# circletile/smvp-toolkit

Measured on AMD Instinct MI355X. Metric: fp64 CSR SpMV GFLOP/s (2*nnz flop per product; achieved HBM GB/s in roofline), higher is better.
Workload: dtype f64; 1 GPU; memplus.mtx x944 block-diagonal (substitute for the SURVEY 8(d) random model; that model: roofline.frac_sur...; format=csr, kernel=csr_stream_owner<8, 5, false>, nnz=119085600, rows=16763552, exchange=none

## Files before the change

### smvp-toolkit_amd/csrc/smvp_kernels.hip

```cpp
#include "smvp_kernels.h"

#include <algorithm>
#include <cstdio>
#include <cstdlib>

namespace smvp {

template <int WIDTH>
__device__ __forceinline__ double shfl_down_sum(double v)
{
#pragma unroll
    for (int off = WIDTH / 2; off > 0; off >>= 1)
        v += __shfl_down(v, off, WIDTH);
    return v;
}


#ifndef SMVP_TU_ILP
template <int T>
__global__ __launch_bounds__(kVectorBlock) void csr_vector_rows(
    const int *__restrict__ row_ptr, const int *__restrict__ col_ind, const double *__restrict__ val,
    const double *__restrict__ x, double *__restrict__ y, int rows, int row0)
{
    const long long gid = (long long)blockIdx.x * kVectorBlock + threadIdx.x;
    const long long row = row0 + gid / T;
    const int lane = threadIdx.x & (T - 1);
    int a = 0, z = 0;
    if (row < rows) {
        a = row_ptr[row];
        z = row_ptr[row + 1];
    }
    double acc = 0.0;
    for (int j = a + lane; j < z; j += T)
        acc += val[j] * x[col_ind[j]];
    acc = shfl_down_sum<T>(acc);
    if (lane == 0 && row < rows)
        y[row] = acc;
}

template <int VPT>
__global__ __launch_bounds__(kStreamBlock) void csr_stream_tiles(
    const int *__restrict__ row_ptr, const int *__restrict__ col_ind, const double *__restrict__ val,
    const double *__restrict__ x, double *__restrict__ y, const int *__restrict__ tile_row,
    double *__restrict__ carry, int rows, int nnz, int ntiles, int tile_group)
{
    constexpr int TILE = kStreamBlock * VPT;
    constexpr int QCAP = TILE / kLongRow + 1;
    __shared__ double prod[TILE];
    __shared__ int long_rows[QCAP];
    __shared__ int long_count;

    const int b = tile_of_block(blockIdx.x, tile_group);
    if (b >= ntiles)
        return;
    const int t = threadIdx.x;
    const long long s = (long long)b * TILE;
    const int e = (int)(s + TILE < (long long)nnz ? s + TILE : (long long)nnz);
    if (t == 0)
        long_count = 0;
    const int rlo = tile_row[b];
    const int rhi = tile_row[b + 1];

    const long long j0 = s + (long long)t * VPT;
    double p[VPT];
    if (j0 + VPT <= (long long)nnz) {
        int c[VPT];
        double v[VPT];
#pragma unroll
        for (int k = 0; k < VPT; k += 4)
            *reinterpret_cast<int4 *>(&c[k]) = *reinterpret_cast<const int4 *>(col_ind + j0 + k);
#pragma unroll
        for (int k = 0; k < VPT; k += 2)
            *reinterpret_cast<double2 *>(&v[k]) = *reinterpret_cast<const double2 *>(val + j0 + k);
#pragma unroll
        for (int k = 0; k < VPT; ++k)
            p[k] = v[k] * x[c[k]];
    } else {
#pragma unroll
        for (int k = 0; k < VPT; ++k)
            p[k] = (j0 + k < (long long)nnz) ? val[j0 + k] * x[col_ind[j0 + k]] : 0.0;
    }
#pragma unroll
    for (int k = 0; k < VPT; k += 2)
        *reinterpret_cast<double2 *>(&prod[t * VPT + k]) = make_double2(p[k], p[k + 1]);
    __syncthreads();

    const int lo = (int)s;
    if (t < 64) {
        const int first = rlo < rows ? row_ptr[rlo] : nnz;
        const int head = (first < e ? first : e) - lo;
        double acc = 0.0;
        for (int i = t; i < head; i += 64)
            acc += prod[i];
        acc = shfl_down_sum<64>(acc);
        if (t == 0)
            carry[b] = acc;
    }

    for (int r = rlo + t; r < rhi; r += kStreamBlock) {
        const int a = row_ptr[r];
        const int nxt = row_ptr[r + 1];
        const int z = nxt < e ? nxt : e;
        if (z - a <= kLongRow) {
            double acc = 0.0;
            for (int i = a - lo; i < z - lo; ++i)
                acc += prod[i];
            y[r] = acc;
        } else {
            long_rows[atomicAdd(&long_count, 1)] = r;
        }
    }
    __syncthreads();

    const int nlong = long_count;
    const int lane = t & 63;
    for (int q = t >> 6; q < nlong; q += kStreamBlock / 64) {
        const int r = long_rows[q];
        const int a = row_ptr[r];
        const int nxt = row_ptr[r + 1];
        const int z = nxt < e ? nxt : e;
        double acc = 0.0;
        for (int i = a - lo + lane; i < z - lo; i += 64)
            acc += prod[i];
        acc = shfl_down_sum<64>(acc);
        if (lane == 0)
            y[r] = acc;
    }
}

#endif
typedef int int4v __attribute__((ext_vector_type(4)));

struct OwnerExtra {
    const int *pos = nullptr;
    const int *start_pos = nullptr;
    const int *ovf_ptr = nullptr;
    const double *ovf_val = nullptr;
    const int *ovf_k = nullptr;
    const int *cache_ptr = nullptr;
    const double *val_cache = nullptr;
    const unsigned short *col16 = nullptr;
    const int *col_base = nullptr;
    const unsigned *word32 = nullptr;
    const unsigned short *group_run = nullptr;
    const int *run_ptr = nullptr;
    const int *run_tab = nullptr;
    int unit_x = 0;
    const unsigned short *row_rel = nullptr;
    unsigned long long *stamps = nullptr;
    int back_grid = 0;
};

[[maybe_unused]] static inline OwnerExtra owner_extra_of(const OwnerLaunch &l, unsigned long long *stamps)
{
    OwnerExtra ex{};
    ex.pos = l.pos, ex.start_pos = l.start_pos, ex.ovf_ptr = l.ovf_ptr, ex.ovf_val = l.ovf_val, ex.ovf_k = l.ovf_k;
    ex.cache_ptr = l.cache_ptr, ex.val_cache = l.val_cache;
    ex.col16 = l.col16, ex.col_base = l.col_base;
    ex.unit_x = l.unit_x, ex.word32 = l.word32, ex.group_run = l.group_run, ex.run_ptr = l.run_ptr, ex.run_tab = l.run_tab;
    ex.row_rel = l.row_rel;
    ex.stamps = stamps;
    return ex;
}

struct OwnerArgs {
    const int *__restrict__ col_ind;
    const double *__restrict__ val;
    const double *__restrict__ x;
    const int *__restrict__ pos;
    const int *__restrict__ start_pos;
    const double *__restrict__ ovf_val;
    const int *__restrict__ ovf_k;
    int unit_x;
};

template <int FLAVOR>
__device__ __forceinline__ double owner_product_slow(const OwnerArgs &a, long long j)
{
    if constexpr (FLAVOR == kFlavorCsr || FLAVOR == kFlavorCsr16)
        return a.val[j] * a.x[a.col_ind[j]];
    else if constexpr (FLAVOR == kFlavorTjdsK)
        return a.val[a.pos[j]] * a.x[a.col_ind[j]];
    else {
        const int p = a.pos[j];
        return a.val[p] * a.x[p - a.start_pos[(unsigned)a.col_ind[j] >> kSlotBits]];
    }
}

template <int FLAVOR>
__device__ __forceinline__ double owner_overflow_product(const OwnerArgs &a, int ovf_base, int e, int i)
{
    if constexpr (FLAVOR == kFlavorTjdsS || FLAVOR == kFlavorTjdsH)
        return a.unit_x ? a.val[a.ovf_k[ovf_base + i]] : a.ovf_val[ovf_base + i] * a.x[a.ovf_k[ovf_base + i]];
    else
        return owner_product_slow<FLAVOR>(a, (long long)e + i);
}

#if defined(SMVP_PHASE_STAMPS) && defined(SMVP_TU_ILP)
#undef SMVP_PHASE_STAMPS
#define SMVP_ILP_UNIT_UNUSED
#endif
#ifdef SMVP_PHASE_STAMPS
__device__ unsigned long long g_owner_phase[8];
#define SMVP_PHASE(n)                                                                        \
    do {                                                                                     \
        if (threadIdx.x == 0 && (blockIdx.x & 127) == 5) {                                   \
            const unsigned long long now_ = wall_clock64();                                  \
            if ((n) > 0)                                                                     \
                atomicAdd(&g_owner_phase[(n)-1], now_ - phase_prev_);                        \
            else                                                                             \
                atomicAdd(&g_owner_phase[7], 1ull);                                          \
            phase_prev_ = now_;                                                              \
        }                                                                                    \
    } while (0)
#else
#define SMVP_PHASE(n) do { } while (0)
#endif

#ifndef SMVP_TJDS_NEUTRALISE
#define SMVP_TJDS_NEUTRALISE 0
#endif

template <int VPT, int FLAVOR, bool STAMPED>
__device__ __forceinline__ void owner_body(
    const int *__restrict__ row_ptr, const int *__restrict__ col_ind, const double *__restrict__ val,
    const double *__restrict__ x, double *__restrict__ y, const int *__restrict__ tile_row,
    const int *__restrict__ tile_next, int rows, int nnz_arg, int ntiles, int tile_group_arg, const OwnerExtra &ex, const int block)
{
    const OwnerArgs a = {col_ind, val, x, ex.pos, ex.start_pos, ex.ovf_val, ex.ovf_k, FLAVOR == kFlavorTjdsH ? ex.unit_x : 0};
    constexpr int TILE = kStreamBlock * VPT;
    constexpr int QCAP = (TILE + kStreamOver) / kLongRow + 1;
    constexpr bool CSR = FLAVOR == kFlavorCsr || FLAVOR == kFlavorCsr16;
    constexpr bool COL16 = FLAVOR == kFlavorCsr16;
    constexpr bool HALF = FLAVOR == kFlavorTjdsH;
    constexpr bool TJDS = FLAVOR == kFlavorTjdsK || FLAVOR == kFlavorTjdsS || HALF;
    constexpr bool SORTED = FLAVOR == kFlavorTjdsS || HALF;
    static_assert(TILE <= (1 << kSlotBits), "slot bits");
    __shared__ double prod[TILE + kStreamOver];
    __shared__ int long_rows[QCAP];
    __shared__ int long_a[QCAP];
    __shared__ int long_z[QCAP];
    __shared__ int long_count;
    __shared__ double wave_sum[kStreamBlock / 64];

    const int t = threadIdx.x;
#ifdef SMVP_PHASE_STAMPS
    unsigned long long phase_prev_ = 0;
#endif
    unsigned long long *stamp = nullptr;
    if constexpr (STAMPED) {
        stamp = ex.stamps + 2 * ((size_t)block * (kStreamBlock / 64) + (t >> 6));
        if ((t & 63) == 0)
            stamp[0] = wall_clock64();
    }
#define SMVP_OWNER_EXIT()                                         \
    do {                                                          \
        if constexpr (STAMPED) {                                  \
            asm volatile("s_waitcnt vmcnt(0)" ::: "memory");      \
            if ((t & 63) == 0)                                    \
                stamp[1] = wall_clock64();                        \
        }                                                         \
        return;                                                   \
    } while (0)

    const int b = tile_of_block_swept(block, tile_group_arg, ex.back_grid);
    if (b >= ntiles)
        SMVP_OWNER_EXIT();
    const int nnz = nnz_arg;
    const long long s = (long long)b * TILE;
    const long long j0 = s + (long long)t * VPT;

    const bool whole = j0 + VPT <= (long long)nnz;
    int c[VPT];
    int pj[VPT];
    double v[VPT];
    const bool full_tile = s + TILE <= (long long)nnz;
    int grp[HALF ? VPT : 1];
    int run0 = 0;
    int2 run_tbl = make_int2(0, 0);
    if constexpr (HALF) {
        if (full_tile) {
            run0 = ex.run_ptr[b];
            const int nruns = ex.run_ptr[b + 1] - run0;
            const int ln = t & 63;
            if (ln < nruns)
                run_tbl = reinterpret_cast<const int2 *>(ex.run_tab)[run0 + ln];
        }
    }
    if constexpr (HALF) {
        if (full_tile) {
#pragma unroll
            for (int k = 0; k < VPT; ++k) {
                if constexpr (VPT == 1) {
                    pj[k] = (int)ex.word32[s + k * kStreamBlock + t];
                } else {
                    pj[k] = (int)__builtin_nontemporal_load(ex.word32 + s + k * kStreamBlock + t);
                }
                const unsigned gw = reinterpret_cast<const unsigned *>(ex.group_run)[((size_t)b * (TILE / 32) + k * (kStreamBlock / 32) +
                                                                                     2 * __builtin_amdgcn_readfirstlane(t >> 6)) >> 1];
                grp[k] = (t & 32) ? (int)(gw >> 16) : (int)(gw & 0xffffu);
            }
        }
    } else if constexpr (SORTED) {
        if (full_tile) {
#pragma unroll
            for (int k = 0; k < VPT; ++k) {
                if constexpr (VPT > 1) {
                    pj[k] = __builtin_nontemporal_load(a.pos + s + k * kStreamBlock + t);
                    c[k] = __builtin_nontemporal_load(a.col_ind + s + k * kStreamBlock + t);
                } else {
                    pj[k] = a.pos[s + k * kStreamBlock + t];
                    c[k] = a.col_ind[s + k * kStreamBlock + t];
                }
            }
        }
    } else if (whole) {
        if constexpr (VPT >= 4) {
            if constexpr (COL16) {
                const int base = ex.col_base[b];
                if (base >= 0) {
#pragma unroll
                    for (int k = 0; k < VPT; k += 4) {
                        const uint2 w = *reinterpret_cast<const uint2 *>(ex.col16 + j0 + k);
                        c[k] = base + (int)(w.x & 0xffffu), c[k + 1] = base + (int)(w.x >> 16);
                        c[k + 2] = base + (int)(w.y & 0xffffu), c[k + 3] = base + (int)(w.y >> 16);
                    }
                } else {
#pragma unroll
                    for (int k = 0; k < VPT; k += 4)
                        *reinterpret_cast<int4 *>(&c[k]) = *reinterpret_cast<const int4 *>(a.col_ind + j0 + k);
                }
            } else {
#pragma unroll
                for (int k = 0; k < VPT; k += 4)
                    *reinterpret_cast<int4 *>(&c[k]) = *reinterpret_cast<const int4 *>(a.col_ind + j0 + k);
            }
            if constexpr (TJDS) {
#pragma unroll
                for (int k = 0; k < VPT; k += 4)
                    *reinterpret_cast<int4v *>(&pj[k]) = __builtin_nontemporal_load(reinterpret_cast<const int4v *>(a.pos + j0 + k));
            }
            if constexpr (CSR) {
#pragma unroll
                for (int k = 0; k < VPT; k += 2)
                    *reinterpret_cast<double2 *>(&v[k]) = *reinterpret_cast<const double2 *>(a.val + j0 + k);
            }
        } else {
            c[0] = a.col_ind[j0];
            if constexpr (TJDS)
                pj[0] = a.pos[j0];
            if constexpr (CSR)
                v[0] = a.val[j0];
        }
    }
    const int rlo = tile_row[b];
    const int rhi = tile_row[b + 1];
    if (rlo == rhi)
        SMVP_OWNER_EXIT();
    SMVP_PHASE(0);
    const int lo = (int)s;
    const int e = (int)(s + TILE < (long long)nnz ? s + TILE : (long long)nnz);
    const int zend = tile_next[b];
    const int ext = zend - e;
    const unsigned short *__restrict__ row_rel = ex.row_rel;
    auto row_bounds = [&](int r, int &ra, int &rz) {
        if (row_rel) {
            ra = row_rel[r];
            rz = r + 1 < rhi ? (int)row_rel[r + 1] : zend - lo;
        } else {
            ra = row_ptr[r] - lo;
            rz = row_ptr[r + 1] - lo;
        }
    };
    const bool giant = ext > kStreamOver;
    if (t == 0)
        long_count = 0;
    const bool over0 = !giant && t < ext;
    double p[VPT];
    double po = 0.0;
    int rp_a = 0, rp_b = 0, rp_a2 = 0, rp_b2 = 0;
    int ovf_base = 0, cache0 = 0, in_place = 0;
    if constexpr (SORTED) {
        ovf_base = ex.ovf_ptr[b];
        cache0 = ex.cache_ptr[b];
        in_place = (e - lo) - (ex.cache_ptr[b + 1] - cache0);
    }
    if constexpr (SORTED) {
        if (full_tile && rlo + t < rhi)
            row_bounds(rlo + t, rp_a, rp_b);
        if (full_tile && rlo + t + kStreamBlock < rhi)
            row_bounds(rlo + t + kStreamBlock, rp_a2, rp_b2);
        int co = 0;
        double vo = 0.0;
        const bool unit_x = HALF && ex.unit_x;
        if (over0 && !(SMVP_TJDS_NEUTRALISE & 8)) {
            co = a.ovf_k[ovf_base + t];
            if (!unit_x)
                vo = a.ovf_val[ovf_base + t];
        }
        if (full_tile) {
            int slot[VPT];
#pragma unroll
            for (int k = 0; k < VPT; ++k) {
                if constexpr (HALF)
                    c[k] = (int)((unsigned)pj[k] >> 16), pj[k] &= 0xffff;
                slot[k] = c[k] & ((1 << kSlotBits) - 1);
                if constexpr (HALF) {
                    const int r = grp[k] + (((c[k] >> kSlotBits) - grp[k]) & 31);
                    int base = __shfl(run_tbl.x, r & 63), sub = __shfl(run_tbl.y, r & 63);
                    if (r >= 64) {
                        const int2 w = reinterpret_cast<const int2 *>(ex.run_tab)[run0 + r];
                        base = w.x, sub = w.y;
                    }
                    pj[k] += base;
                    c[k] = pj[k] - sub;
                } else {
                    c[k] = pj[k] - a.start_pos[(unsigned)c[k] >> kSlotBits];
                }
            }
            double xk[VPT];
#pragma unroll
            for (int k = 0; k < VPT; ++k) {
                const int idx = k * kStreamBlock + t;
                const double *src = idx < in_place ? a.val + pj[k] : ex.val_cache + (cache0 + (idx - in_place));
                if ((SMVP_TJDS_NEUTRALISE & 2) && idx < in_place)
                    v[k] = 1.0;
                else if ((SMVP_TJDS_NEUTRALISE & 4) && idx >= in_place)
                    v[k] = 1.0;
                else
                    v[k] = *src;
            }
            double xo = 0.0;
            if (unit_x) {
#pragma unroll
                for (int k = 0; k < VPT; ++k)
                    xk[k] = 1.0;
                if (over0)
                    vo = a.val[co], xo = 1.0;
            } else {
#pragma unroll
                for (int k = 0; k < VPT; ++k)
                    xk[k] = (SMVP_TJDS_NEUTRALISE & 1) ? 1.0 : a.x[c[k]];
                xo = over0 && !(SMVP_TJDS_NEUTRALISE & 8) ? a.x[co] : 0.0;
            }
#pragma unroll
            for (int k = 0; k < VPT; ++k)
                prod[slot[k]] = v[k] * xk[k];
            po = vo * xo;
        } else {
            for (int k = 0; k < VPT; ++k) {
                const int idx = k * kStreamBlock + t;
                if (s + idx < (long long)nnz) {
                    if constexpr (HALF) {
                        const unsigned w32 = ex.word32[s + idx];
                        const int m = (int)(w32 >> 16), g = ex.group_run[(size_t)b * (TILE / 32) + (idx >> 5)];
                        const int r = g + (((m >> kSlotBits) - g) & 31);
                        const int2 w = reinterpret_cast<const int2 *>(ex.run_tab)[ex.run_ptr[b] + r];
                        const int pw = w.x + (int)(w32 & 0xffffu);
                        const double vv = idx < in_place ? a.val[pw] : ex.val_cache[cache0 + (idx - in_place)];
                        prod[m & ((1 << kSlotBits) - 1)] = unit_x ? vv : vv * a.x[pw - w.y];
                    } else {
                        const int pw = a.pos[s + idx];
                        const double vv = idx < in_place ? a.val[pw] : ex.val_cache[cache0 + (idx - in_place)];
                        const int m = a.col_ind[s + idx];
                        prod[m & ((1 << kSlotBits) - 1)] = vv * a.x[pw - a.start_pos[(unsigned)m >> kSlotBits]];
                    }
                }
            }
            if (over0)
                po = unit_x ? a.val[co] : vo * a.x[co];
        }
    } else if (whole) {
        if (rlo + t < rhi)
            row_bounds(rlo + t, rp_a, rp_b);
        if (rlo + t + kStreamBlock < rhi)
            row_bounds(rlo + t + kStreamBlock, rp_a2, rp_b2);
        int co = 0, pjo = 0;
        double vo = 0.0;
        if (over0) {
            co = a.col_ind[e + t];
            if constexpr (TJDS)
                pjo = a.pos[e + t];
            if constexpr (CSR)
                vo = a.val[e + t];
        }
        double xk[VPT];
        if constexpr (TJDS) {
#pragma unroll
            for (int k = 0; k < VPT; ++k)
                v[k] = a.val[pj[k]];
            if (over0)
                vo = a.val[pjo];
        }
#pragma unroll
        for (int k = 0; k < VPT; ++k)
            xk[k] = a.x[c[k]];
        const double xo = over0 ? a.x[co] : 0.0;
#pragma unroll
        for (int k = 0; k < VPT; ++k)
            p[k] = v[k] * xk[k];
        po = vo * xo;
    } else {
#pragma unroll
        for (int k = 0; k < VPT; ++k)
            p[k] = (j0 + k < (long long)nnz) ? owner_product_slow<FLAVOR>(a, j0 + k) : 0.0;
        if (over0)
            po = owner_product_slow<FLAVOR>(a, e + t);
    }
    if constexpr (!SORTED) {
        if constexpr (VPT >= 2) {
#pragma unroll
            for (int k = 0; k < VPT; k += 2)
                *reinterpret_cast<double2 *>(&prod[t * VPT + k]) = make_double2(p[k], p[k + 1]);
        } else {
            prod[t] = p[0];
        }
    }
    if (over0)
        prod[e - lo + t] = po;
    if (!giant)
        for (int i = t + kStreamBlock; i < ext; i += kStreamBlock)
            prod[e - lo + i] = owner_overflow_product<FLAVOR>(a, ovf_base, e, i);
    SMVP_PHASE(1);
    __syncthreads();
    SMVP_PHASE(2);

    const int last = rhi - 1;
    auto finish_row = [&](int r, int ra, int rz) {
        if (rz - ra <= kLongRow) {
            double acc = 0.0;
            for (int i = ra; i < rz; i += 4) {
                const double v0 = prod[i], v1 = prod[i + 1 < rz ? i + 1 : i], v2 = prod[i + 2 < rz ? i + 2 : i],
                             v3 = prod[i + 3 < rz ? i + 3 : i];
                acc += v0;
                if (i + 1 < rz)
                    acc += v1;
                if (i + 2 < rz)
                    acc += v2;
                if (i + 3 < rz)
                    acc += v3;
            }
            if constexpr (VPT == 1)
                y[r] = acc;
            else
                __builtin_nontemporal_store(acc, &y[r]);
        } else {
            const int q = atomicAdd(&long_count, 1);
            long_rows[q] = r;
            long_a[q] = ra;
            long_z[q] = rz;
        }
    };
    int r_next = rlo + t;
    if (full_tile) {
        if (r_next < rhi && !(giant && r_next == last))
            finish_row(r_next, rp_a, rp_b);
        r_next += kStreamBlock;
        if (r_next < rhi && !(giant && r_next == last))
            finish_row(r_next, rp_a2, rp_b2);
        r_next += kStreamBlock;
    }
    for (int r = r_next; r < rhi; r += kStreamBlock) {
        if (giant && r == last)
            continue;
        int ra, rz;
        row_bounds(r, ra, rz);
        finish_row(r, ra, rz);
    }
    SMVP_PHASE(3);
    __syncthreads();
    SMVP_PHASE(4);

    const int nlong = long_count;
    const int lane = t & 63;
    for (int q = t >> 6; q < nlong; q += kStreamBlock / 64) {
        const int zq = long_z[q];
        double acc = 0.0;
        for (int i = long_a[q] + lane; i < zq; i += 64)
            acc += prod[i];
        acc = wave_sum_dpp(acc);
        if (lane == 0)
            y[long_rows[q]] = acc;
    }
    SMVP_PHASE(5);

    if (giant) {
        const int ra = row_ptr[last];
        double acc = 0.0;
        for (int i = ra - lo + t; i < e - lo; i += kStreamBlock)
            acc += prod[i];
        for (int j = e + t; j < zend; j += 4 * kStreamBlock) {
            double pg[4];
#pragma unroll
            for (int u = 0; u < 4; ++u) {
                const int jj = j + u * kStreamBlock;
                pg[u] = jj < zend ? owner_overflow_product<FLAVOR>(a, ovf_base, e, jj - e) : 0.0;
            }
#pragma unroll
            for (int u = 0; u < 4; ++u)
                acc += pg[u];
        }
        acc = shfl_down_sum<64>(acc);
        if (lane == 0)
            wave_sum[t >> 6] = acc;
        __syncthreads();
        if (t == 0) {
            double total = 0.0;
#pragma unroll
            for (int w = 0; w < kStreamBlock / 64; ++w)
                total += wave_sum[w];
            y[last] = total;
        }
    }
    SMVP_OWNER_EXIT();
#undef SMVP_OWNER_EXIT
}

template <int VPT, int FLAVOR, bool STAMPED>
__global__ __launch_bounds__(kStreamBlock) void csr_stream_owner(
    const int *__restrict__ row_ptr, const int *__restrict__ col_ind, const double *__restrict__ val,
    const double *__restrict__ x, double *__restrict__ y, const int *__restrict__ tile_row,
    const int *__restrict__ tile_next, int rows, int nnz_arg, int ntiles, int tile_group_arg, const OwnerExtra ex)
{
    owner_body<VPT, FLAVOR, STAMPED>(row_ptr, col_ind, val, x, y, tile_row, tile_next, rows, nnz_arg, ntiles, tile_group_arg, ex,
                                     (int)blockIdx.x);
}

#ifndef SMVP_TU_ILP
constexpr int kRepeatMaxShards = 32;
constexpr unsigned kRepeatAbort = 0x80000000u;

struct RepeatCtl {
    unsigned *sticky = nullptr;
    unsigned *shard = nullptr;
    unsigned *top = nullptr;
    unsigned *go = nullptr;
    unsigned long long *stamps = nullptr;
    int reps = 0, grid_virtual = 0, slots_per_product = 0;
    int shards = 1;
    unsigned long long patience = 0;
};

template <int VPT, int FLAVOR>
__global__ __launch_bounds__(kStreamBlock) void csr_stream_owner_repeat(
    const int *__restrict__ row_ptr, const int *__restrict__ col_ind, const double *__restrict__ val,
    const double *__restrict__ x, double *__restrict__ y, const int *__restrict__ tile_row,
    const int *__restrict__ tile_next, int rows, int nnz_arg, int ntiles, int tile_group_arg, const OwnerExtra ex, const RepeatCtl ctl)
{
    __shared__ unsigned go;
    const int t = threadIdx.x;
    const unsigned nwg = gridDim.x, me = blockIdx.x;
    const unsigned S = (unsigned)ctl.shards;
    const unsigned sh = me % S;
    const unsigned members = (nwg - sh + S - 1) / S;
    const unsigned arrivals = S > 1 ? (nwg < S ? nwg : S) : nwg;
    unsigned long long *stamp = ctl.stamps + 2 * ((size_t)me * (kStreamBlock / 64) + (t >> 6));
    if (t == 0) {
        go = __hip_atomic_load(ctl.sticky, __ATOMIC_RELAXED, __HIP_MEMORY_SCOPE_AGENT) ? 0u : 1u;
        if (!go)
            atomicOr(ctl.top, kRepeatAbort);
    }
    __syncthreads();
    if (!go)
        return;
    for (int rep = 0; rep < ctl.reps; ++rep) {
        __syncthreads();
        if (t == 0) {
            const unsigned gen = (unsigned)rep + 1u;
            const unsigned long long t0 = wall_clock64();
            unsigned seen = 0;
            if (S > 1) {
                const unsigned before = atomicAdd(ctl.shard + 32 * sh, 1u);
                if (before + 1u == members * gen) {
                    const unsigned tb = atomicAdd(ctl.top, 1u);
                    if ((tb & ~kRepeatAbort) + 1u == arrivals * gen)
                        for (unsigned q = 0; q < S; ++q)
                            __hip_atomic_fetch_max(ctl.go + 32 * q, gen, __ATOMIC_RELAXED, __HIP_MEMORY_SCOPE_AGENT);
                }
                for (;;) {
                    const unsigned g = __hip_atomic_load(ctl.go + 32 * sh, __ATOMIC_RELAXED, __HIP_MEMORY_SCOPE_AGENT);
                    if (g >= gen && g != kRepeatAbort)
                        break;
                    if (g == kRepeatAbort) {
                        seen = kRepeatAbort;
                        break;
                    }
                    if (wall_clock64() - t0 > ctl.patience) {
                        atomicOr(ctl.top, kRepeatAbort);
                        __hip_atomic_store(ctl.sticky, 1u, __ATOMIC_RELAXED, __HIP_MEMORY_SCOPE_AGENT);
                        for (unsigned q = 0; q < S; ++q)
                            __hip_atomic_fetch_max(ctl.go + 32 * q, kRepeatAbort, __ATOMIC_RELAXED, __HIP_MEMORY_SCOPE_AGENT);
                        seen = kRepeatAbort;
                        break;
                    }
                    __builtin_amdgcn_s_sleep(2);
                }
            } else {
                atomicAdd(ctl.top, 1u);
                for (;;) {
                    seen = __hip_atomic_load(ctl.top, __ATOMIC_RELAXED, __HIP_MEMORY_SCOPE_AGENT);
                    if ((seen & kRepeatAbort) || (seen & ~kRepeatAbort) >= arrivals * gen)
                        break;
                    if (wall_clock64() - t0 > ctl.patience) {
                        atomicOr(ctl.top, kRepeatAbort);
                        __hip_atomic_store(ctl.sticky, 1u, __ATOMIC_RELAXED, __HIP_MEMORY_SCOPE_AGENT);
                        seen = kRepeatAbort;
                        break;
                    }
                    __builtin_amdgcn_s_sleep(1);
                }
            }
            go = seen & kRepeatAbort ? 0u : 1u;
        }
        __syncthreads();
        if (!go)
            return;
        if ((t & 63) == 0)
            stamp[0] = wall_clock64();
        for (int vb = (int)me; vb < ctl.grid_virtual; vb += (int)nwg) {
            if (vb != (int)me)
                __syncthreads();
            owner_body<VPT, FLAVOR, false>(row_ptr, col_ind, val, x, y, tile_row, tile_next, rows, nnz_arg, ntiles, tile_group_arg, ex, vb);
        }
        asm volatile("s_waitcnt vmcnt(0)" ::: "memory");
        if ((t & 63) == 0)
            stamp[1] = wall_clock64();
        stamp += 2 * (size_t)ctl.slots_per_product;
    }
}

__global__ __launch_bounds__(256) void stamp_reduce(const unsigned long long *__restrict__ stamps, int slots_per_product,
                                                    unsigned long long *__restrict__ first_last)
{
    __shared__ unsigned long long lo_s[256 / 64], hi_s[256 / 64];
    const unsigned long long *s = stamps + (size_t)blockIdx.x * slots_per_product * 2;
    unsigned long long lo = ~0ull, hi = 0ull;
    for (int i = threadIdx.x; i < slots_per_product; i += 256) {
        const unsigned long long f = s[2 * i], l = s[2 * i + 1];
        lo = f < lo ? f : lo;
        hi = l > hi ? l : hi;
    }
#pragma unroll
    for (int off = 32; off > 0; off >>= 1) {
        const unsigned long long ol = __shfl_down(lo, off, 64), oh = __shfl_down(hi, off, 64);
        lo = ol < lo ? ol : lo;
        hi = oh > hi ? oh : hi;
    }
    if ((threadIdx.x & 63) == 0) {
        lo_s[threadIdx.x >> 6] = lo;
        hi_s[threadIdx.x >> 6] = hi;
    }
    __syncthreads();
    if (threadIdx.x == 0) {
        for (int w = 1; w < 256 / 64; ++w) {
            lo = lo_s[w] < lo ? lo_s[w] : lo;
            hi = hi_s[w] > hi ? hi_s[w] : hi;
        }
        first_last[2 * blockIdx.x] = lo;
        first_last[2 * blockIdx.x + 1] = hi;
    }
}

__global__ __launch_bounds__(256) void csr_stream_carry_fixup(
    const int *__restrict__ carry_row, const double *__restrict__ carry, double *__restrict__ y, int ntiles)
{
    const int b = blockIdx.x * 256 + threadIdx.x;
    if (b >= ntiles)
        return;
    const int r = carry_row[b];
    if (r < 0 || (b > 0 && carry_row[b - 1] == r))
        return;
    double acc = y[r];
    for (int k = b; k < ntiles && carry_row[k] == r; ++k)
        acc += carry[k];
    y[r] = acc;
}

template <bool OPERAND_BY_ROW>
__global__ __launch_bounds__(kTjdsBlock) void tjds_colmajor_scatter(
    const int *__restrict__ start_pos, const int *__restrict__ row_ind, const double *__restrict__ val,
    const double *__restrict__ x_perm, double *__restrict__ y, const int4 *__restrict__ work, int cols)
{
    const int4 w = work[blockIdx.x];
    const int k = w.x + threadIdx.x;
    const double xk = (!OPERAND_BY_ROW && k < cols) ? x_perm[k] : 0.0;
    int r[kTjdsDiagChunk];
    double v[kTjdsDiagChunk];
#pragma unroll
    for (int i = 0; i < kTjdsDiagChunk; ++i) {
        const int d = w.y + i;
        r[i] = -1;
        v[i] = 0.0;
        if (d < w.z) {
            const int base = start_pos[d];
            if (k < start_pos[d + 1] - base) {
                r[i] = row_ind[base + k];
                v[i] = val[base + k];
            }
        }
    }
#pragma unroll
    for (int i = 0; i < kTjdsDiagChunk; ++i) {
        if (r[i] >= 0) {
            const double xv = OPERAND_BY_ROW ? x_perm[r[i]] : xk;
            unsafeAtomicAdd(&y[r[i]], v[i] * xv);
        }
    }
}

__global__ __launch_bounds__(kTjdsBlock) void tjds_colmajor_products(
    const int *__restrict__ start_pos, const double *__restrict__ val, const double *__restrict__ x_perm,
    double *__restrict__ prod, const int4 *__restrict__ work, int cols)
{
    const int4 w = work[blockIdx.x];
    const int k = w.x + threadIdx.x;
    const double xk = k < cols ? x_perm[k] : 0.0;
    int j[kTjdsDiagChunk];
    double v[kTjdsDiagChunk];
#pragma unroll
    for (int i = 0; i < kTjdsDiagChunk; ++i) {
        const int d = w.y + i;
        j[i] = -1;
        v[i] = 0.0;
        if (d < w.z) {
            const int base = start_pos[d];
            if (k < start_pos[d + 1] - base) {
                j[i] = base + k;
                v[i] = val[base + k];
            }
        }
    }
#pragma unroll
    for (int i = 0; i < kTjdsDiagChunk; ++i)
        if (j[i] >= 0)
            __builtin_nontemporal_store(v[i] * xk, &prod[j[i]]);
}

__global__ __launch_bounds__(256) void tjds_permute_operand(
    const int *__restrict__ perm, const double *__restrict__ x, double *__restrict__ x_perm, int cols)
{
    const int k = blockIdx.x * 256 + threadIdx.x;
    if (k < cols)
        x_perm[k] = x[perm[k]];
}

__global__ __launch_bounds__(256) void find_out_of_range(const int *__restrict__ a, long long n, int limit,
                                                          int *__restrict__ bad)
{
    const long long stride = (long long)gridDim.x * 256;
    for (long long i = (long long)blockIdx.x * 256 + threadIdx.x; i < n; i += stride) {
        const int v = a[i];
        if (v < 0 || v >= limit)
            atomicMax(bad, (int)(i < 2147483646ll ? i + 1 : 2147483647ll));
    }
}

__global__ __launch_bounds__(256) void vector_absmax(const double *__restrict__ v, long long n,
                                                      unsigned long long *__restrict__ bits)
{
    double m = 0.0;
    const long long stride = (long long)gridDim.x * 256;
    for (long long i = (long long)blockIdx.x * 256 + threadIdx.x; i < n; i += stride) {
        const double a = fabs(v[i]);
// ... 579 lines not shown
```

Baseline: 885.8 GFLOP/s.

## Reorder owner-kernel loads to issue index, row bounds, values before gathers

For non-sorted flavors with VPT other than 4, the owner kernel now issues tile metadata, index words, row-pointer bounds (raw, rebased later) and the overflow element loads first, then values, then the x gathers, with scheduling barriers that keep this order. It also prefetches a third row's bounds when VPT is at least 8 and removes the over0 branch around the overflow load by clamping its index to e-1. The aim is to get more independent memory requests in flight before the dependent x gathers, hiding HBM latency. In exchange it raises register pressure and may lower occupancy, and it adds a special path that zeroes y when nnz is 0.

```diff
diff --git a/smvp-toolkit_amd/csrc/smvp_kernels.hip b/smvp-toolkit_amd/csrc/smvp_kernels.hip
--- a/smvp-toolkit_amd/csrc/smvp_kernels.hip
+++ b/smvp-toolkit_amd/csrc/smvp_kernels.hip
@@ -235,6 +235,8 @@
     constexpr bool HALF = FLAVOR == kFlavorTjdsH;
     constexpr bool TJDS = FLAVOR == kFlavorTjdsK || FLAVOR == kFlavorTjdsS || HALF;
     constexpr bool SORTED = FLAVOR == kFlavorTjdsS || HALF;
+    constexpr bool GROUPED = !SORTED && VPT != 4;
+    constexpr bool THIRD_ROW = GROUPED && VPT >= 8;
     static_assert(TILE <= (1 << kSlotBits), "slot bits");
     __shared__ double prod[TILE + kStreamOver];
     __shared__ int long_rows[QCAP];
@@ -267,6 +269,13 @@
     if (b >= ntiles)
         SMVP_OWNER_EXIT();
     const int nnz = nnz_arg;
+    if constexpr (GROUPED) {
+        if (nnz == 0) {
+            for (int r = t; r < rows; r += kStreamBlock)
+                y[r] = 0.0;
+            SMVP_OWNER_EXIT();
+        }
+    }
     const long long s = (long long)b * TILE;
     const long long j0 = s + (long long)t * VPT;
 
@@ -274,7 +283,15 @@
     int c[VPT];
     int pj[VPT];
     double v[VPT];
+    [[maybe_unused]] unsigned raw16[COL16 ? VPT / 2 : 1];
     const bool full_tile = s + TILE <= (long long)nnz;
+    int rlo = 0, rhi = 0, zend = 0;
+    [[maybe_unused]] int base16 = 0;
+    if constexpr (GROUPED) {
+        rlo = tile_row[b], rhi = tile_row[b + 1], zend = tile_next[b];
+        if constexpr (COL16)
+            base16 = ex.col_base[b];
+    }
     int grp[HALF ? VPT : 1];
     int run0 = 0;
     int2 run_tbl = make_int2(0, 0);
@@ -314,21 +331,14 @@
                 }
             }
         }
-    } else if (whole) {
+    }
+    [[maybe_unused]] auto load_index_words = [&]() {
         if constexpr (VPT >= 4) {
             if constexpr (COL16) {
-                const int base = ex.col_base[b];
-                if (base >= 0) {
-#pragma unroll
-                    for (int k = 0; k < VPT; k += 4) {
-                        const uint2 w = *reinterpret_cast<const uint2 *>(ex.col16 + j0 + k);
-                        c[k] = base + (int)(w.x & 0xffffu), c[k + 1] = base + (int)(w.x >> 16);
-                        c[k + 2] = base + (int)(w.y & 0xffffu), c[k + 3] = base + (int)(w.y >> 16);
-                    }
-                } else {
-#pragma unroll
-                    for (int k = 0; k < VPT; k += 4)
-                        *reinterpret_cast<int4 *>(&c[k]) = *reinterpret_cast<const int4 *>(a.col_ind + j0 + k);
+#pragma unroll
+                for (int k = 0; k < VPT; k += 4) {
+                    const uint2 w = *reinterpret_cast<const uint2 *>(ex.col16 + j0 + k);
+                    raw16[k / 2] = w.x, raw16[k / 2 + 1] = w.y;
                 }
             } else {
 #pragma unroll
@@ -339,37 +349,72 @@
 #pragma unroll
                 for (int k = 0; k < VPT; k += 4)
                     *reinterpret_cast<int4v *>(&pj[k]) = __builtin_nontemporal_load(reinterpret_cast<const int4v *>(a.pos + j0 + k));
-            }
-            if constexpr (CSR) {
-#pragma unroll
-                for (int k = 0; k < VPT; k += 2)
-                    *reinterpret_cast<double2 *>(&v[k]) = *reinterpret_cast<const double2 *>(a.val + j0 + k);
             }
         } else {
             c[0] = a.col_ind[j0];
             if constexpr (TJDS)
                 pj[0] = a.pos[j0];
-            if constexpr (CSR)
-                v[0] = a.val[j0];
-        }
-    }
-    const int rlo = tile_row[b];
-    const int rhi = tile_row[b + 1];
+        }
+    };
+    if constexpr (!SORTED && !GROUPED) {
+        if (whole) {
+            if constexpr (VPT >= 4) {
+                if constexpr (COL16) {
+                    const int base = ex.col_base[b];
+                    if (base >= 0) {
+#pragma unroll
+                        for (int k = 0; k < VPT; k += 4) {
+                            const uint2 w = *reinterpret_cast<const uint2 *>(ex.col16 + j0 + k);
+                            c[k] = base + (int)(w.x & 0xffffu), c[k + 1] = base + (int)(w.x >> 16);
+                            c[k + 2] = base + (int)(w.y & 0xffffu), c[k + 3] = base + (int)(w.y >> 16);
+                        }
+                    } else {
+#pragma unroll
+                        for (int k = 0; k < VPT; k += 4)
+                            *reinterpret_cast<int4 *>(&c[k]) = *reinterpret_cast<const int4 *>(a.col_ind + j0 + k);
+                    }
+                } else {
+#pragma unroll
+                    for (int k = 0; k < VPT; k += 4)
+                        *reinterpret_cast<int4 *>(&c[k]) = *reinterpret_cast<const int4 *>(a.col_ind + j0 + k);
+                }
+                if constexpr (TJDS) {
+#pragma unroll
+                    for (int k = 0; k < VPT; k += 4)
+                        *reinterpret_cast<int4v *>(&pj[k]) = __builtin_nontemporal_load(reinterpret_cast<const int4v *>(a.pos + j0 + k));
+                }
+                if constexpr (CSR) {
+#pragma unroll
+                    for (int k = 0; k < VPT; k += 2)
+                        *reinterpret_cast<double2 *>(&v[k]) = *reinterpret_cast<const double2 *>(a.val + j0 + k);
+                }
+            } else {
+                c[0] = a.col_ind[j0];
+                if constexpr (TJDS)
+                    pj[0] = a.pos[j0];
+                if constexpr (CSR)
+                    v[0] = a.val[j0];
+            }
+        }
+    }
+    if constexpr (!GROUPED)
+        rlo = tile_row[b], rhi = tile_row[b + 1];
     if (rlo == rhi)
         SMVP_OWNER_EXIT();
     SMVP_PHASE(0);
     const int lo = (int)s;
     const int e = (int)(s + TILE < (long long)nnz ? s + TILE : (long long)nnz);
-    const int zend = tile_next[b];
+    if constexpr (!GROUPED)
+        zend = tile_next[b];
     const int ext = zend - e;
     const unsigned short *__restrict__ row_rel = ex.row_rel;
-    auto row_bounds = [&](int r, int &ra, int &rz) {
+    auto row_bounds = [&](int r, int &ra, int &rz, bool raw = false) {
         if (row_rel) {
             ra = row_rel[r];
             rz = r + 1 < rhi ? (int)row_rel[r + 1] : zend - lo;
         } else {
-            ra = row_ptr[r] - lo;
-            rz = row_ptr[r + 1] - lo;
+            ra = row_ptr[r] - (raw ? 0 : lo);
+            rz = row_ptr[r + 1] - (raw ? 0 : lo);
         }
     };
     const bool giant = ext > kStreamOver;
@@ -379,6 +424,7 @@
     double p[VPT];
     double po = 0.0;
     int rp_a = 0, rp_b = 0, rp_a2 = 0, rp_b2 = 0;
+    [[maybe_unused]] int rp_a3 = 0, rp_b3 = 0;
     int ovf_base = 0, cache0 = 0, in_place = 0;
     if constexpr (SORTED) {
         ovf_base = ex.ovf_ptr[b];
@@ -470,42 +516,122 @@
             if (over0)
                 po = unit_x ? a.val[co] : vo * a.x[co];
         }
-    } else if (whole) {
-        if (rlo + t < rhi)
-            row_bounds(rlo + t, rp_a, rp_b);
-        if (rlo + t + kStreamBlock < rhi)
-            row_bounds(rlo + t + kStreamBlock, rp_a2, rp_b2);
-        int co = 0, pjo = 0;
-        double vo = 0.0;
-        if (over0) {
-            co = a.col_ind[e + t];
+    } else if constexpr (!GROUPED) {
+        if (whole) {
+            if (rlo + t < rhi)
+                row_bounds(rlo + t, rp_a, rp_b);
+            if (rlo + t + kStreamBlock < rhi)
+                row_bounds(rlo + t + kStreamBlock, rp_a2, rp_b2);
+            int co = 0, pjo = 0;
+            double vo = 0.0;
+            if (over0) {
+                co = a.col_ind[e + t];
+                if constexpr (TJDS)
+                    pjo = a.pos[e + t];
+                if constexpr (CSR)
+                    vo = a.val[e + t];
+            }
+            double xk[VPT];
+            if constexpr (TJDS) {
+#pragma unroll
+                for (int k = 0; k < VPT; ++k)
+                    v[k] = a.val[pj[k]];
+                if (over0)
+                    vo = a.val[pjo];
+            }
+#pragma unroll
+            for (int k = 0; k < VPT; ++k)
+                xk[k] = a.x[c[k]];
+            const double xo = over0 ? a.x[co] : 0.0;
+#pragma unroll
+            for (int k = 0; k < VPT; ++k)
+                p[k] = v[k] * xk[k];
+            po = vo * xo;
+        } else {
+#pragma unroll
+            for (int k = 0; k < VPT; ++k)
+                p[k] = (j0 + k < (long long)nnz) ? owner_product_slow<FLAVOR>(a, j0 + k) : 0.0;
+            if (over0)
+                po = owner_product_slow<FLAVOR>(a, e + t);
+        }
+    } else {
+        double xk[VPT];
+        double vo = 0.0, xo = 0.0;
+        if (whole) {
+            load_index_words();
+            if (rlo + t < rhi)
+                row_bounds(rlo + t, rp_a, rp_b, true);
+            if (rlo + t + kStreamBlock < rhi)
+                row_bounds(rlo + t + kStreamBlock, rp_a2, rp_b2, true);
+            if constexpr (THIRD_ROW) {
+                if (rlo + t + 2 * kStreamBlock < rhi)
+                    row_bounds(rlo + t + 2 * kStreamBlock, rp_a3, rp_b3, true);
+            }
+            const int jo = over0 ? e + t : e - 1;
+            const int co = a.col_ind[jo];
+            int pjo = 0;
             if constexpr (TJDS)
-                pjo = a.pos[e + t];
-            if constexpr (CSR)
-                vo = a.val[e + t];
-        }
-        double xk[VPT];
-        if constexpr (TJDS) {
-#pragma unroll
-            for (int k = 0; k < VPT; ++k)
-                v[k] = a.val[pj[k]];
-            if (over0)
-                vo = a.val[pjo];
-        }
-#pragma unroll
-        for (int k = 0; k < VPT; ++k)
-            xk[k] = a.x[c[k]];
-        const double xo = over0 ? a.x[co] : 0.0;
+                pjo = a.pos[jo];
+            __builtin_amdgcn_sched_barrier(0);
+            if constexpr (CSR) {
+                if constexpr (VPT >= 4) {
+#pragma unroll
+                    for (int k = 0; k < VPT; k += 2)
+                        *reinterpret_cast<double2 *>(&v[k]) = *reinterpret_cast<const double2 *>(a.val + j0 + k);
+                } else {
+                    v[0] = a.val[j0];
+                }
+                vo = a.val[jo];
+            }
+            __builtin_amdgcn_sched_barrier(0);
+            auto gathers = [&]() {
+                if constexpr (TJDS) {
+#pragma unroll
+                    for (int k = 0; k < VPT; ++k)
+                        v[k] = a.val[pj[k]];
+                }
+#pragma unroll
+                for (int k = 0; k < VPT; ++k)
+                    xk[k] = a.x[c[k]];
+                if constexpr (TJDS)
+                    vo = a.val[pjo];
+                xo = a.x[co];
+            };
+            if constexpr (COL16) {
+                if (base16 < 0) {
+#pragma unroll
+                    for (int k = 0; k < VPT; k += 4)
+                        *reinterpret_cast<int4 *>(&c[k]) = *reinterpret_cast<const int4 *>(a.col_ind + j0 + k);
+                    gathers();
+                    __builtin_amdgcn_sched_barrier(0);
+                } else {
+#pragma unroll
+                    for (int k = 0; k < VPT; k += 2)
+                        c[k] = base16 + (int)(raw16[k / 2] & 0xffffu), c[k + 1] = base16 + (int)(raw16[k / 2] >> 16);
+                    gathers();
+                }
+            } else {
+                gathers();
+            }
+            if (!row_rel)
+                rp_a -= lo, rp_b -= lo, rp_a2 -= lo, rp_b2 -= lo, rp_a3 -= lo, rp_b3 -= lo;
+        } else {
+#pragma unroll
+            for (int k = 0; k < VPT; ++k) {
+                v[k] = 0.0, xk[k] = 0.0;
+                if (j0 + k < (long long)nnz) {
+                    if constexpr (CSR)
+                        v[k] = a.val[j0 + k];
+                    else
+                        v[k] = a.val[a.pos[j0 + k]];
+                    xk[k] = a.x[a.col_ind[j0 + k]];
+                }
+            }
+        }
 #pragma unroll
         for (int k = 0; k < VPT; ++k)
             p[k] = v[k] * xk[k];
-        po = vo * xo;
-    } else {
-#pragma unroll
-        for (int k = 0; k < VPT; ++k)
-            p[k] = (j0 + k < (long long)nnz) ? owner_product_slow<FLAVOR>(a, j0 + k) : 0.0;
-        if (over0)
-            po = owner_product_slow<FLAVOR>(a, e + t);
+        po = over0 ? vo * xo : 0.0;
     }
     if constexpr (!SORTED) {
         if constexpr (VPT >= 2) {
@@ -559,6 +685,11 @@
         if (r_next < rhi && !(giant && r_next == last))
             finish_row(r_next, rp_a2, rp_b2);
         r_next += kStreamBlock;
+        if constexpr (THIRD_ROW) {
+            if (r_next < rhi && !(giant && r_next == last))
+                finish_row(r_next, rp_a3, rp_b3);
+            r_next += kStreamBlock;
+        }
     }
     for (int r = r_next; r < rhi; r += kStreamBlock) {
         if (giant && r == last)
```

Result: no change. 893.8 GFLOP/s (median of 6 runs) (+0.9%).
